# 1pathplanningzzj/pointnet_refine

Measured on AMD Instinct MI355X. Metric: lane segments/sec (fwd+bwd) at B=4096,N=1024; HBM GB/s vs roofline, higher is better.
Workload: dtype f32 (large GEMMs: 2xfp16-split MFMA, 3 products, fp32 accumulate); 1 GPU; LineRefineNet training step (fwd + deep-supervision L1 + bwd + Adam), B=4096/GPU, N=1024, M=32, C=4; global_batch=4096, points=1024, parallelism=dp1, decoder_chunk=4096

## Files before the change

include/pointnet_refine_hip.h:

```cpp
#ifndef POINTNET_REFINE_HIP_H
#define POINTNET_REFINE_HIP_H

#include <stddef.h>
#include <stdint.h>

#ifdef __cplusplus
extern "C" {
#endif

#define PRH_OK 0
#define PRH_ERR_ARG (-1)
#define PRH_ERR_WORKSPACE (-2)
#define PRH_ERR_HIP (-3)

#define PRH_MAX_LAYERS 8

typedef struct {
  const float* w;
  const float* b;
  const float* gamma;
  const float* beta;
  float* running_mean;
  float* running_var;
  int64_t* num_batches_tracked;
// ... 442 lines not shown
int prh_add_dropout_layernorm_forward(const float* x, const float* r, const float* gamma, const float* beta,
                                      long rows, int channels, float eps, float dropout_p, unsigned seed,
                                      float* y, float* mean, float* rstd, int device, void* stream);
size_t prh_add_dropout_layernorm_workspace_bytes(void);
int prh_add_dropout_layernorm_backward(const float* dy, const float* x, const float* r, const float* gamma,
                                       const float* mean, const float* rstd, long rows, int channels,
                                       float dropout_p, unsigned seed, float* dx, float* dr, float* dgamma,
                                       float* dbeta, void* workspace, size_t workspace_bytes, int device,
                                       void* stream);

size_t prh_l1_loss_workspace_bytes(void);
int prh_l1_loss(const float* pred, const float* target, int n_layers, long elems, double denom,
                int accumulate, float* loss, float* d_pred, float* geometry, double points,
                void* workspace, size_t workspace_bytes, int device, void* stream);

int prh_adam_step(float* param, const float* grad, float* exp_avg, float* exp_avg_sq, long n, float lr,
                  float beta1, float beta2, float eps, float weight_decay, int step, int device,
                  void* stream);

int prh_attn_backward_ex(const float* q, long ldq, const float* k, long ldk, const float* v, long ldv,
                         const float* o, long ldo, const float* lse, const float* dout, long lddo,
                         float* dq, long lddq, float* dk, long lddk, float* dv, long lddv, int B, int M,
                         int N, int H, float scale, float dropout_p, unsigned seed, float* kv_amax_part,
                         int device, void* stream);

int prh_set_gemm_mode(int mode);
int prh_get_gemm_mode(void);

int prh_set_dropout_seed_source(const unsigned* device_word);

int prh_test_gemm_nt(const float* a, const float* w, float* c, int m, int n, int k,
                     void* workspace, size_t workspace_bytes, int device, void* stream);
size_t prh_test_gemm_tn_workspace_bytes(int p, int mo, int ni);
size_t prh_test_gate_backward_workspace_bytes(int out_dim);
int prh_test_gate_backward(const float* ctx, int B, int N, int in_channel, int out_dim, const float* gate_w1,
                           const float* gate_b1, const float* gate_w2, const float* gate_b2, const float* z_fus,
                           const float* bn_scale, const float* bn_shift, float* d_fused, float* gate, int recompute,
                           float* ws_a, float* ws_b, void* workspace, size_t workspace_bytes, int device, void* stream);
int prh_test_gemm_tn(const float* a, const float* b, float* c, float* colsum, int p, int mo,
                     int ni, void* workspace, size_t workspace_bytes, int device, void* stream);
size_t prh_test_gemm_tn_side_workspace_bytes(int p, int mo, int ni);
int prh_test_gemm_tn_side(const float* a, const float* b, float* c, float* colsum, int p, int mo,
                          int ni, float* dy, long lddy, const float* z, long ldz, const float* ka,
                          const float* kb, const float* kc, long rows, int cols, int side,
                          float* amax_out, void* workspace, size_t workspace_bytes, int device,
                          void* stream);
int prh_test_gemm_tn_side_ex(const float* a, const float* b, float* c, float* colsum, int p, int mo,
                             int ni, const float* qa, const float* qb, float* dy, long lddy,
                             const float* z, long ldz, const float* ka, const float* kb,
                             const float* kc, long rows, int cols, int side, int period,
                             int* period_used, float* amax_out, void* workspace,
                             size_t workspace_bytes, int device, void* stream);

enum {
  PRH_REDUCE_SLABS = 0, PRH_REDUCE_BN_STAGE1 = 1, PRH_REDUCE_PARTIALS = 2, PRH_REDUCE_LN_PARAM_GRAD = 3,
  PRH_REDUCE_FINAL = 4, PRH_REDUCE_ACT_AMAX = 5
};
int prh_test_reduce_depth(int kind);
int prh_test_reduce_slabs(const float* slab, int s, int rows, int cols, float* out, long ldout,
                          const float* cslab, int ccols, float* cout, int device, void* stream);
int prh_test_reduce_bn_stage1(const float* ws_a, const float* ws_b, int r, long ld, int n,
                              int tile_rows, int p, int forward, double* out, int device,
                              void* stream);
int prh_test_reduce_partials(const float* ws_a, const float* ws_b, int r2, int n, float* out_a,
                             float* out_b, int device, void* stream);
int prh_test_reduce_ln_param_grad(const float* part_g, const float* part_b, int nb, float* dgamma,
// ... 25 lines not shown
```

pointnet_refine_amd/_lib.py:

```python
from __future__ import annotations

import ctypes as C
import os
import subprocess
import threading

_HERE = os.path.dirname(os.path.abspath(__file__))
_ROOT = os.path.dirname(_HERE)
LIB_PATH = os.environ.get("PRH_LIB_PATH") or os.path.join(_HERE, "libpointnet_refine_hip.so")
_CSRC = os.path.join(_HERE, "csrc")
_SOURCES = [os.path.join(_CSRC, "prh_lib.hip")] + (sorted(
    os.path.join(_CSRC, f) for f in os.listdir(_CSRC) if f.endswith((".hpp", ".h", ".hip")) and f != "prh_lib.hip")
    if os.path.isdir(_CSRC) else [])
_HEADER = os.path.join(_ROOT, "include", "pointnet_refine_hip.h")

PRH_MAX_LAYERS = 8


class BnLayer(C.Structure):
    _fields_ = [("w", C.c_void_p), ("b", C.c_void_p), ("gamma", C.c_void_p), ("beta", C.c_void_p),
                ("running_mean", C.c_void_p), ("running_var", C.c_void_p),
                ("num_batches_tracked", C.c_void_p), ("cin", C.c_int), ("cout", C.c_int)]


# ... 11 lines not shown
    _fields_ = [("conv", BnLayerGrad * 5), ("fusion", BnLayerGrad), ("d_gate_w1", C.c_void_p),
                ("d_gate_b1", C.c_void_p), ("d_gate_w2", C.c_void_p), ("d_gate_b2", C.c_void_p)]


class EncoderSaved(C.Structure):
    _fields_ = [("z_cat", C.c_void_p), ("z_fus", C.c_void_p), ("gate", C.c_void_p),
                ("bn_scale", C.c_void_p), ("bn_shift", C.c_void_p), ("bn_mean", C.c_void_p),
                ("bn_rstd", C.c_void_p), ("argmax", C.c_void_p), ("op_amax", C.c_void_p),
                ("gate_recompute", C.c_int)]


class EncoderSavedBf16(C.Structure):
    _fields_ = [("z_cat", C.c_void_p), ("z_fus", C.c_void_p), ("gate", C.c_void_p),
                ("bn_scale", C.c_void_p), ("bn_shift", C.c_void_p), ("bn_mean", C.c_void_p),
                ("bn_rstd", C.c_void_p), ("argmax", C.c_void_p)]


EXPORTS = [
    "prh_encoder_workspace_bytes", "prh_encoder_gate_recompute", "prh_encoder_forward", "prh_encoder_backward",
    "prh_encoder_bf16_workspace_bytes", "prh_encoder_forward_bf16", "prh_encoder_backward_bf16",
    "prh_linear_bf16_workspace_bytes", "prh_linear_forward_bf16", "prh_linear_backward_bf16",
    "prh_linear_forward_out16", "prh_linear_backward_dy16", "prh_attn_forward_kv16", "prh_attn_backward_kv16",
    "prh_encoder_fused_image_bytes", "prh_encoder_fused_prepare", "prh_encoder_fused_workspace_bytes",
    "prh_encoder_fused_forward",
    "prh_linear_forward_workspace_bytes", "prh_linear_forward", "prh_linear_forward_ex",
    "prh_linear_forward_full", "prh_linear_forward_amax", "prh_operand_absmax_workspace_bytes", "prh_operand_absmax",
    "prh_linear_uses_operand_maxima", "prh_linear_backward_full", "prh_linear_backward_amax", "prh_pos_hidden_forward",
    "prh_pos_hidden_forward_workspace_bytes", "prh_pos_hidden_forward_amax", "prh_pos_hidden_backward_workspace_bytes",
    "prh_pos_hidden_backward", "prh_linear_small_forward", "prh_linear_small_backward_workspace_bytes",
    "prh_linear_small_backward",
    "prh_linear_backward_workspace_bytes", "prh_linear_backward", "prh_linear_backward_ex",
    "prh_mlp_stack_workspace_bytes", "prh_mlp_stack_forward", "prh_mlp_stack_backward",
    "prh_test_gemm_nt", "prh_test_gemm_tn_workspace_bytes", "prh_test_gemm_tn",
    "prh_test_gate_backward_workspace_bytes", "prh_test_gate_backward",
    "prh_test_gemm_tn_side_workspace_bytes", "prh_test_gemm_tn_side", "prh_test_gemm_tn_side_ex", "prh_test_xcc_map",
    "prh_test_reduce_depth", "prh_test_reduce_slabs", "prh_test_reduce_bn_stage1", "prh_test_reduce_partials",
    "prh_test_reduce_ln_param_grad", "prh_test_reduce_pos_hidden_final", "prh_test_reduce_partial_rows_final",
    "prh_test_reduce_act_amax_workspace_bytes", "prh_test_reduce_act_amax",
    "prh_profile_enable", "prh_profile_count", "prh_profile_reset", "prh_profile_read",
    "prh_attn_forward", "prh_attn_backward", "prh_attn_backward_ex",
    "prh_context_workspace_bytes", "prh_context_build",
    "prh_context_ragged_workspace_bytes", "prh_context_ragged_count", "prh_context_ragged_select",
    "prh_line_metrics", "prh_shift_sweep_workspace_bytes", "prh_shift_sweep",
    "prh_shift_sweep_ragged_workspace_bytes", "prh_shift_sweep_ragged",
    "prh_drive_slice_workspace_bytes", "prh_drive_slice_count", "prh_drive_slice_write",
    "prh_drive_clip_workspace_bytes", "prh_drive_clip_count", "prh_drive_clip_write",
    "prh_drive_noise_workspace_bytes", "prh_drive_noise",
    "prh_match_clip_workspace_bytes", "prh_match_clip_count", "prh_match_clip_write",
    "prh_match_costs_workspace_bytes", "prh_match_costs", "prh_match_max_side", "prh_match_assign",
    "prh_bev_bounds_workspace_bytes", "prh_bev_bounds", "prh_bev_raster", "prh_bev_select_workspace_bytes",
    "prh_bev_select", "prh_bev_tone", "prh_bev_colorize", "prh_bev_crop", "prh_bev_tile", "prh_bev_draw_count",
    "prh_bev_draw_workspace_bytes", "prh_bev_draw",
    "prh_view_bounds_workspace_bytes", "prh_view_bounds", "prh_view_clear", "prh_view_max_views", "prh_view_splat",
    "prh_view_lines", "prh_view_resolve",
    "prh_fuse_max_points", "prh_fuse_tile", "prh_fuse_project_workspace_bytes", "prh_fuse_project",
    "prh_fuse_gather_workspace_bytes", "prh_fuse_gather",
    "prh_link_tile", "prh_link_pairs_per_block", "prh_link_pairs_workspace_bytes", "prh_link_pairs_count",
    "prh_link_pairs_write", "prh_link_stats",
    "prh_link_cum", "prh_link_edges_blocks", "prh_link_edges", "prh_link_edges_compact", "prh_link_label_round",
    "prh_link_tree_init", "prh_link_tree_level",
    "prh_support_max_cells", "prh_support_accumulate",
    "prh_ground_max_bins", "prh_ground_bin_workspace_bytes", "prh_ground_bin_count", "prh_ground_bin_write",
    "prh_ground_query",
    "prh_align_tile", "prh_align_max_shifts", "prh_align_select_workspace_bytes", "prh_align_select_count",
    "prh_align_select_write", "prh_align_score",
    "prh_align_max_poses", "prh_align_select_cells_workspace_bytes", "prh_align_select_cells_count",
# ... 298 lines not shown
    lib.prh_add_dropout_layernorm_backward.argtypes = [vp, vp, vp, vp, vp, vp, lg, i, f, C.c_uint, vp, vp, vp, vp,
                                                       vp, C.c_size_t, i, vp]
    lib.prh_l1_loss_workspace_bytes.restype = C.c_size_t
    lib.prh_l1_loss_workspace_bytes.argtypes = []
    lib.prh_l1_loss.restype = i
    lib.prh_l1_loss.argtypes = [vp, vp, i, lg, C.c_double, i, vp, vp, vp, C.c_double, vp, C.c_size_t, i, vp]
    lib.prh_adam_step.restype = i
    lib.prh_adam_step.argtypes = [vp, vp, vp, vp, lg, f, f, f, f, f, i, i, vp]
    lib.prh_cast_perm_bf16.restype = i
    lib.prh_cast_perm_bf16.argtypes = [vp, lg, vp, lg, i, vp]
    lib.prh_posmem_images.restype = i
    lib.prh_posmem_images.argtypes = [vp, lg, vp, vp, vp, vp, vp, lg, lg, vp, vp, i, vp]
    lib.prh_attn_fold_forward.restype = i
    lib.prh_attn_fold_forward.argtypes = [vp, lg, vp, vp, vp, lg, vp, lg, vp, vp, lg, i, i, i, i, C.c_float, i, vp]
    lib.prh_relu_mask_absmax.restype = i
    lib.prh_relu_mask_absmax.argtypes = [vp, vp, vp, lg, f, vp, vp, sz, i, vp]
    lib.prh_set_gemm_mode.restype = i
    lib.prh_set_gemm_mode.argtypes = [i]
    lib.prh_attn_backward_ex.restype = i
    lib.prh_attn_backward_ex.argtypes = [vp, lg, vp, lg, vp, lg, vp, lg, vp, vp, lg, vp, lg, vp, lg, vp, lg,
                                         i, i, i, i, f, f, C.c_uint, vp, i, vp]
    lib.prh_set_dropout_seed_source.restype = i
    lib.prh_set_dropout_seed_source.argtypes = [vp]
    lib.prh_get_gemm_mode.restype = i
    lib.prh_profile_enable.restype = i
    lib.prh_profile_enable.argtypes = [i]
    lib.prh_profile_count.restype = i
    lib.prh_profile_reset.restype = i
    lib.prh_profile_read.restype = i
    lib.prh_profile_read.argtypes = [i, C.c_char_p, i, C.POINTER(C.c_float), C.POINTER(C.c_double),
                                     C.POINTER(C.c_double)]
    lib.prh_test_gemm_nt.restype = i
    lib.prh_test_gemm_nt.argtypes = [vp, vp, vp, i, i, i, vp, sz, i, vp]
    lib.prh_test_gate_backward_workspace_bytes.restype = sz
    lib.prh_test_gate_backward_workspace_bytes.argtypes = [i]
    lib.prh_test_gate_backward.restype = i
    lib.prh_test_gate_backward.argtypes = [vp, i, i, i, i, vp, vp, vp, vp, vp, vp, vp, vp, vp, i, vp, vp, vp, sz, i, vp]
    lib.prh_test_gemm_tn_workspace_bytes.restype = sz
    lib.prh_test_gemm_tn_workspace_bytes.argtypes = [i, i, i]
    lib.prh_test_gemm_tn.restype = i
    lib.prh_test_gemm_tn.argtypes = [vp, vp, vp, vp, i, i, i, vp, sz, i, vp]
    lib.prh_test_gemm_tn_side_workspace_bytes.restype = sz
    lib.prh_test_gemm_tn_side_workspace_bytes.argtypes = [i, i, i]
    lib.prh_test_gemm_tn_side.restype = i
    lib.prh_test_gemm_tn_side.argtypes = [vp, vp, vp, vp, i, i, i, vp, lg, vp, lg, vp, vp, vp, lg, i, i, vp, vp, sz, i, vp]
    lib.prh_test_gemm_tn_side_ex.restype = i
    lib.prh_test_gemm_tn_side_ex.argtypes = [vp, vp, vp, vp, i, i, i, vp, vp, vp, lg, vp, lg, vp, vp, vp, lg, i, i, i,
                                             C.POINTER(i), vp, vp, sz, i, vp]
    lib.prh_test_xcc_map.restype = i
    lib.prh_test_xcc_map.argtypes = [i, i, vp, i, vp]
    if not hasattr(lib, "prh_test_reduce_depth"):
        return lib
    lib.prh_test_reduce_depth.restype = i
    lib.prh_test_reduce_depth.argtypes = [i]
    lib.prh_test_reduce_slabs.restype = i
    lib.prh_test_reduce_slabs.argtypes = [vp, i, i, i, vp, lg, vp, i, vp, i, vp]
    lib.prh_test_reduce_bn_stage1.restype = i
    lib.prh_test_reduce_bn_stage1.argtypes = [vp, vp, i, lg, i, i, i, i, vp, i, vp]
    lib.prh_test_reduce_partials.restype = i
    lib.prh_test_reduce_partials.argtypes = [vp, vp, i, i, vp, vp, i, vp]
    lib.prh_test_reduce_ln_param_grad.restype = i
    lib.prh_test_reduce_ln_param_grad.argtypes = [vp, vp, i, vp, vp, i, vp]
    lib.prh_test_reduce_pos_hidden_final.restype = i
    lib.prh_test_reduce_pos_hidden_final.argtypes = [vp, i, i, vp, vp, i, vp]
    lib.prh_test_reduce_partial_rows_final.restype = i
    lib.prh_test_reduce_partial_rows_final.argtypes = [vp, i, i, vp, i, vp, i, vp]
# ... 80 lines not shown
```

pointnet_refine_amd/csrc/prh_gemm_h2.hpp:

```cpp
#pragma once
#include "prh_gemm_s3.hpp"

namespace prh {

constexpr int H2_BK = 32;
constexpr int H2_PLANE = 256 * H2_BK * 2;
constexpr int H2_OPER = 2 * H2_PLANE;
constexpr int H2_STAGE = 2 * H2_OPER;
constexpr int H2_LDS = 2 * H2_STAGE;

__device__ __forceinline__ int h2_off(int row, int k) {
  return row * 64 + ((((k >> 3) ^ (-(row >> 2))) & 3) << 4) + ((k & 7) << 1);
}

inline size_t h2_weight_bytes(int N, int K) {
  return S3_WHDR + (size_t)((N + 255) / 256) * ((K + H2_BK - 1) / H2_BK) * H2_OPER;
}

__global__ __launch_bounds__(256) void prep_weights_h2_kernel(const float* __restrict__ W, int N,
                                                              int K, long ldw, char* __restrict__ out,
                                                              const float* __restrict__ amax) {
  const int KT = (K + H2_BK - 1) / H2_BK;
  const int NT_ = (N + 255) / 256;
  const long total = (long)NT_ * 256 * KT * 4;
// ... 292 lines not shown
      for (int r = 0; r < 4; ++r) acc[i][j][r] *= unscale;
  if constexpr (AMAX) {
    float wmax = 0.f;
    nt_epilogue_vec<EPI, 4, f32x4[8][4], false, true>(acc, p, m0 + wm, n0 + wn, tile_m * 2 + (wave >> 2), lane,
                                                       reinterpret_cast<float*>(smem) + wave * (32 * EPI_LDW), false, &wmax);
    __syncthreads();
    float* red = reinterpret_cast<float*>(smem);
    if (lane == 0) red[wave] = wmax;
    __syncthreads();
    if (tid == 0)
      p.ws_a[blockIdx.x] = fmaxf(fmaxf(fmaxf(red[0], red[1]), fmaxf(red[2], red[3])),
                                 fmaxf(fmaxf(red[4], red[5]), fmaxf(red[6], red[7])));
  } else if constexpr (EPI == EPI_GATE_BWD) {
    static_assert(8 * (32 + 16) * EPI_LDW * 4 <= H2_LDS, "gate-backward scratch must fit in the stage buffers");
    nt_epilogue_vec<EPI, 4>(acc, p, m0 + wm, n0 + wn, tile_m * 2 + (wave >> 2), lane,
                            reinterpret_cast<float*>(smem) + wave * (32 * EPI_LDW), false, nullptr,
                            reinterpret_cast<float*>(smem) + 8 * (32 * EPI_LDW) + wave * (16 * EPI_LDW));
  } else {
    nt_epilogue_vec<EPI, 4>(acc, p, m0 + wm, n0 + wn, tile_m * 2 + (wave >> 2), lane,
                            reinterpret_cast<float*>(smem) + wave * (32 * EPI_LDW));
  }
#ifdef PRH_STAMP
  PRH_TICK(2)
  asm volatile("s_waitcnt vmcnt(0)" ::: "memory");
  PRH_TICK(3)
  const int which = (p.K == 1024 && p.N == 1984) ? 0 : (p.K == 1984 && p.N == 1024) ? 1 : (p.K == 256 && p.N == 1536) ? 2 : (p.K == 512 && p.N == 1024) ? 3 : -1;
  if (g_prh_stamp != nullptr && which >= 0 && blockIdx.x == gridDim.x / 2 + 3 && lane == 0 && (wave & 3) == 0) {
    unsigned* o = g_prh_stamp + 64 + which * 16 + (wave >> 2) * 8;
#pragma unroll
    for (int i = 0; i < 4; ++i) o[i] = t_acc[i];
    o[4] = (unsigned)KT;
  }
#endif
}

typedef __fp16 fp16x4 __attribute__((__vector_size__(4 * sizeof(__fp16))));
constexpr int TR_ROW = 576;
constexpr int TR_PLANE = 16 * TR_ROW;
constexpr int TR_OPER = 2 * TR_PLANE;
constexpr int TR_STAGE = 2 * TR_OPER;
constexpr int TR_LDS = 2 * TR_STAGE;

__device__ __forceinline__ f16x8 tr_fragment(const char* plane, int col0, int lane) {
  const int g = lane >> 4, j = lane & 15;
  const char* a = plane + ((g >> 1) * 8 + (j >> 2)) * TR_ROW + (col0 + (g & 1) * 16 + 4 * (j & 3)) * 2;
  const fp16x4 lo = __builtin_amdgcn_ds_read_tr16_b64_v4f16(
      (__attribute__((address_space(3))) fp16x4*)(a));
  const fp16x4 hi = __builtin_amdgcn_ds_read_tr16_b64_v4f16(
      (__attribute__((address_space(3))) fp16x4*)(a + 4 * TR_ROW));
  struct Pair { fp16x4 a, b; } pr = {lo, hi};
  return __builtin_bit_cast(f16x8, pr);
}

constexpr int TR_PACE = 8;
constexpr int TR_PACE_SPINS = 256;
constexpr int TR_SIDE_MAX_COLS = 4096;
inline size_t tr_side_lds(int cols) { return (size_t)3 * ((cols + 255) / 256 * 256) * 4 + 64; }
typedef unsigned int u32x4 __attribute__((ext_vector_type(4)));

template <int PROB, bool SIDE = false, int Q = 1>
__global__ __launch_bounds__(512, 2) void gemm_tn_tr_kernel(const TNParams p) {
  static_assert(PROB == PRO_NONE || PROB == PRO_BNRELU, "prologue not supported");
  static_assert(Q == 1 || (SIDE && (Q == 2 || Q == 4)), "side period: 1, 2 or 4 k-tiles");
  extern __shared__ __attribute__((aligned(16))) char smem[];
  const int tid = threadIdx.x, lane = tid & 63, wave = tid >> 6;
  const int wm = (wave >> 2) * 128, wn = (wave & 3) * 64;
// ... 282 lines not shown
```

pointnet_refine_amd/csrc/prh_lib.hip:

```cpp
#include "../../include/pointnet_refine_hip.h"

#include <hip/hip_runtime.h>
#include <stdarg.h>
#include <stdio.h>
#include <string.h>

#include <mutex>
#include <vector>

#include <stdlib.h>

#include "prh_gemm.hpp"
#include "prh_attn.hpp"
#include "prh_attn16.hpp"
#include "prh_gemm_s3.hpp"
#include "prh_gemm_h2.hpp"
#include "prh_b16.hpp"
#include "prh_small.hpp"
#include "prh_attnfold.hpp"
#include "prh_fused.hpp"
#include "prh_context.hpp"
#include "prh_metrics.hpp"
#include "prh_drive.hpp"
#include "prh_match.hpp"
#include "prh_bev.hpp"
#include "prh_view.hpp"
#include "prh_fuse.hpp"
#include "prh_link.hpp"
#include "prh_link_sync.hpp"
#include "prh_support.hpp"
#include "prh_ground.hpp"
#include "prh_align.hpp"
#include "prh_trace.hpp"
#include "prh_pcd.hpp"
#include "prh_kernels.hpp"

using namespace prh;

namespace {
// ... 345 lines not shown
  const long tiles = (long)p.tiles_n * cdiv(p.M, TM * 32);
  char nm[64];
  snprintf(nm, sizeof(nm), "gemm_small<%d%d%d,%s,%d> K=%d N=%d", TM, TN, KS, NN ? "nn" : "nt", EPI, p.K, p.N);
  const double by = 4.0 * ((double)p.M * p.K + (double)p.M * p.N * ((p.flags & F_RESID) || EPI == EPI_DGRAD ? 2 : 1) + (double)p.N * p.K);
  ProfScope ps(nm, 2.0 * p.M * (double)p.N * p.K, by, st);
  hipLaunchKernelGGL((gemm_small_kernel<TM, TN, KS, NN, EPI>), dim3((unsigned)tiles), dim3(256), (small_lds<TM, TN, KS>()), st, p);
  LAUNCH_CHECK();
  return PRH_OK;
}
template <bool NN, int EPI = EPI_BIAS>
int launch_small(NTParams& p, hipStream_t st) {
  p.flags &= ~F_POOL;
  const bool n64 = !NN || (p.N & 63) == 0;
  if (n64 && (long)cdiv(p.M, 64) * cdiv(p.N, 64) >= 192) return launch_small_cfg<2, 2, 1, NN, EPI>(p, st);
  if (n64 && (long)cdiv(p.M, 32) * cdiv(p.N, 64) >= 192) return launch_small_cfg<1, 2, 2, NN, EPI>(p, st);
  return launch_small_cfg<1, 1, 4, NN, EPI>(p, st);
}
constexpr int TN_SMALL_MAX_P = 16384;
inline bool small_tn_dims_ok(int P, int Mo, int Ni) {
  return P >= 64 && P <= TN_SMALL_MAX_P && (P & 63) == 0 && (Mo & 63) == 0 && (Ni & 63) == 0;
}
inline void small_tn_plan(int P, int Mo, int Ni, int& splits, int& rps) {
  const int tiles = (Mo / 64) * (Ni / 64), chunks = P / 64;
  int s = cdiv(512, tiles);
  s = s > chunks ? chunks : (s < 1 ? 1 : s);
  rps = cdiv(chunks, s) * 64;
  splits = cdiv(P, rps);
}

inline size_t nt_amax_part_floats(int M, int N) {
  const size_t t = (size_t)cdiv(M < 1 ? 1 : M, S3_BM) * cdiv(N < 1 ? 1 : N, S3_BN);
  return (t > (size_t)ABSMAX_MAX_BLOCKS ? t : (size_t)ABSMAX_MAX_BLOCKS) + 64;
}
template <int PRO, int EPI>
int launch_nt_core(Cores c, NTParams& p, hipStream_t st, StatInfo* si, float* amax_part, long* amax_tiles) {
  if (p.M <= 0 || p.N <= 0) return PRH_OK;
  if ((p.K & 3) || (PRO != PRO_GATE1 && (p.lda & 3)) || (p.ldw & 3) ||
      (PRO == PRO_BNBWD && (p.lda2 & 3)))
    return fail(PRH_ERR_ARG, "gemm_nt: K/lda/ldw must be multiples of 4 (K=%d lda=%ld ldw=%ld)",
                p.K, p.lda, p.ldw);
  if constexpr (PRO == PRO_NONE && EPI == EPI_BIAS) {
    if (c.mode == 4 && c.core == 2 && nt_b16_generic_ok(p)) return launch_nt_b16<PRO_NONE, EPI_BIAS, false, false>(p, st, si);
  }
  const bool want_pool = (p.flags & F_POOL) != 0;
  p.flags &= ~F_POOL;
  char nm[64];
  const double by = 4.0 * ((double)p.M * p.K * (PRO == PRO_BNBWD ? 2 : (PRO == PRO_GATE1 ? 0 : 1)) +
                           (double)p.M * p.N * (EPI == EPI_GATE_BWD ? 4 : (EPI == EPI_GATE ? 3 : (EPI == EPI_DGRAD ? 2 : 1))) +
                           (double)p.N * p.K);
  {
    if (p.wprep != nullptr && nt_use_s3(c, p.M, p.N, p.K) && p.lda <= 65536 && p.lda2 <= 65536 &&
        !((EPI == EPI_GATE || EPI == EPI_GATE_BWD) && ((p.N | (int)p.ldc | (int)p.lde1 | (int)p.ldc2) & 3) != 0)) {
      const int KT = cdiv(p.K, S3_BK), NTl = cdiv(p.N, S3_BN);
      const long th = (long)NTl * 256 * KT * 2;
      float* hdr = reinterpret_cast<float*>(p.wprep);
      const char* img = p.wprep + S3_WHDR;
      if (c.core == 3) {
        if (p.amaxW == nullptr) {
          TRY_RC((measure_absmax<PRO_NONE>(p.W, p.ldw, nullptr, 0, nullptr, nullptr, nullptr, p.N, p.K, hdr, hdr + 64, st)));
          p.amaxW = hdr;
        }
        if (p.amaxA == nullptr) {
          TRY_RC((measure_absmax<PRO>(p.A, p.lda, p.A2, p.lda2, p.pa, p.pb, p.pc, p.M, p.K, hdr + 1, hdr + 64, st)));
          p.amaxA = hdr + 1;
        }
      }
      if constexpr (PRO == PRO_NONE || PRO == PRO_BNRELU || PRO == PRO_GATE1) {
        const bool vec_ok = ((p.N | (int)p.ldc) & 3) == 0 && (p.E1 == nullptr || ((int)p.lde1 & 3) == 0) &&
                            (p.flags & F_E1_ROWVEC) == 0 && (p.C2 == nullptr || ((int)p.ldc2 & 3) == 0);
        const int KT2 = cdiv(p.K, H2_BK);
        const size_t lds = (size_t)H2_LDS + (PRO == PRO_NONE ? 0 : 2 * (size_t)(KT2 + 2) * H2_BK * 4);
        if (c.core == 3 && vec_ok && lds <= 160 * 1024) {
          const long th2 = (long)NTl * 256 * KT2 * 4;
          hipLaunchKernelGGL(prep_weights_h2_kernel, dim3((unsigned)cdiv(th2, 256)), dim3(256), 0, st, p.W,
                             p.N, p.K, p.ldw, p.wprep + S3_WHDR, p.amaxW);
          LAUNCH_CHECK();
          p.tiles_n = NTl;
          if (want_pool) p.flags |= F_POOL;
          static const int attr_h2 = allow_big_lds(gemm_nt_h2_kernel<PRO, EPI>, gemm_nt_h2_kernel<PRO, EPI, true>);
          if (attr_h2 != PRH_OK) return attr_h2;
          snprintf(nm, sizeof(nm), "gemm_nt_h2<%d,%d> K=%d N=%d", PRO, EPI, p.K, p.N);
          ProfScope ps(nm, 2.0 * p.M * (double)p.N * p.K, by, st);
          if constexpr (PRO == PRO_NONE && EPI == EPI_BIAS) {
            if (amax_part != nullptr) {
              static const int attr_am = allow_big_lds(gemm_nt_h2_kernel<PRO, EPI, false, true>);
              if (attr_am != PRH_OK) return attr_am;
              const long wgs = (long)NTl * cdiv(p.M, 256);
              p.ws_a = amax_part;
              hipLaunchKernelGGL((gemm_nt_h2_kernel<PRO, EPI, false, true>), dim3((unsigned)wgs), dim3(512), lds, st, p, img);
              LAUNCH_CHECK();
              *amax_tiles = wgs;
              return PRH_OK;
            }
          }
          if (g_h2_pp)
            hipLaunchKernelGGL((gemm_nt_h2_kernel<PRO, EPI, true>), dim3((unsigned)(NTl * cdiv(p.M, 256))), dim3(512),
                               lds, st, p, img);
          else
            hipLaunchKernelGGL((gemm_nt_h2_kernel<PRO, EPI>), dim3((unsigned)(NTl * cdiv(p.M, 256))), dim3(512),
                               lds, st, p, img);
          LAUNCH_CHECK();
          if (si) { si->count = 2 * cdiv(p.M, S3_BM); si->rows = 128; }
          return PRH_OK;
        }
      }
      if constexpr (EPI != EPI_GATE_BWD) {
        hipLaunchKernelGGL(prep_weights_s3_kernel, dim3((unsigned)cdiv(th, 256)), dim3(256), 0, st,
                           p.W, p.N, p.K, p.ldw, 0, p.wprep + S3_WHDR, c.core == 3 ? p.amaxW : nullptr);
        LAUNCH_CHECK();
        p.tiles_n = NTl;
        const long tiles = (long)NTl * cdiv(p.M, S3_BM);
        static const int attr_rc = allow_big_lds(gemm_nt_s3_kernel<PRO, EPI, 3>, gemm_nt_s3_kernel<PRO, EPI, 1>,
                                                 gemm_nt_s3_kernel<PRO, EPI, 2>);
        if (attr_rc != PRH_OK) return attr_rc;
        snprintf(nm, sizeof(nm), "gemm_nt_%s<%d,%d> K=%d N=%d", c.core == 3 ? "h2g1" : c.tag(), PRO, EPI, p.K, p.N);
// ... 1 lines not shown
        switch (c.core) {
          case 2: launch_nt_s3<PRO, EPI, 1>(p, tiles, img, st); break;
          case 3: launch_nt_s3<PRO, EPI, 2>(p, tiles, img, st); break;
          default: launch_nt_s3<PRO, EPI, 3>(p, tiles, img, st);
        }
        LAUNCH_CHECK();
        if (si) { si->count = 2 * cdiv(p.M, S3_BM); si->rows = 128; }
        return PRH_OK;
      }
    }
  }
  if constexpr (EPI == EPI_GATE_BWD) {
    return fail(PRH_ERR_ARG, "gemm_nt: the gate-recompute backward needs the split-fp16 core (M=%d N=%d)", p.M, p.N);
  } else {
    if constexpr (PRO == PRO_NONE && EPI == EPI_BIAS) {
      if (small_nt_ok(p, false)) return launch_small<false>(p, st);
    }
    p.tiles_n = cdiv(p.N, BN);
    const long tiles = (long)p.tiles_n * cdiv(p.M, BM);
    snprintf(nm, sizeof(nm), "gemm_nt<%d,%d> K=%d N=%d", PRO, EPI, p.K, p.N);
    ProfScope ps(nm, 2.0 * p.M * (double)p.N * p.K, by, st);
    if (p.N <= 64)
      hipLaunchKernelGGL((gemm_nt_kernel<PRO, EPI, true>), dim3((unsigned)tiles), dim3(256), 0, st, p);
    else
      hipLaunchKernelGGL((gemm_nt_kernel<PRO, EPI>), dim3((unsigned)tiles), dim3(256), 0, st, p);
    LAUNCH_CHECK();
    if (si) { si->count = 2 * cdiv(p.M, BM); si->rows = 64; }
    return PRH_OK;
  }
}

template <int PRO, int EPI>
int launch_nt(Cores c, NTParams& p, hipStream_t st, StatInfo* si = nullptr, float* amax_out = nullptr,
              float* amax_part = nullptr) {
  long tiles = 0;
  TRY_RC((launch_nt_core<PRO, EPI>(c, p, st, si, amax_part, &tiles)));
  if (amax_out == nullptr) return PRH_OK;
  if (tiles > 0) {
    hipLaunchKernelGGL(absmax_final_kernel, dim3(1), dim3(256), 0, st, (const float*)amax_part, (int)tiles, amax_out);
    LAUNCH_CHECK();
    return PRH_OK;
  }
  return measure_absmax<PRO_NONE>(p.C, p.ldc, nullptr, 0, nullptr, nullptr, nullptr, p.M, p.N, amax_out, amax_part, st);
}

constexpr int TN_S3_MAX_LD = 4096;
struct TNPlan { int tiles_m, tiles_n, splits, rows_per_split; bool s3; };
inline TNPlan tn_plan(Cores c, int P, int Mo, int Ni, bool allow_s3, long maxld = TN_S3_MAX_LD) {
  TNPlan pl;
  pl.s3 = allow_s3 && tn_use_s3(c, P, Mo, Ni);
  const int tile = pl.s3 ? 256 : 128, bk = pl.s3 ? S3_BK : BK;
  pl.tiles_m = cdiv(Mo, tile);
  pl.tiles_n = cdiv(Ni, tile);
  const int tiles = pl.tiles_m * pl.tiles_n;
  int s = cdiv(pl.s3 ? (P >= 262144 ? 768 : 256) : 1024, tiles);
  if (pl.s3) {
    int best = s; double bw = 1e9;
    for (int c = (s > 3 ? s - 2 : 1); c <= s + 4; ++c) {
      const double blocks = (double)tiles * c, w = (double)cdiv((long)blocks, 256L) * 256.0 / blocks;
      if (w < bw - 1e-3) { bw = w; best = c; }
    }
    s = best;
  }
  const int minrows = pl.s3 ? 512 : 128;
  const int smax = cdiv(P, minrows) < 1 ? 1 : cdiv(P, minrows);
  if (s > smax) s = smax;
  if (s < 1) s = 1;
  int rps = cdiv(P, s);
  rps = cdiv(rps, bk) * bk;
// ... 3428 lines not shown
  }
  g_prof.on = true;
  return PRH_OK;
}
int prh_profile_count(void) {
  std::lock_guard<std::mutex> lk(g_prof.mu);
  return (int)g_prof.used;
}
int prh_profile_reset(void) {
  std::lock_guard<std::mutex> lk(g_prof.mu);
  g_prof.used = 0;
  return PRH_OK;
}
int prh_profile_read(int i, char* name, int name_len, float* ms, double* flops, double* bytes) {
  std::lock_guard<std::mutex> lk(g_prof.mu);
  if (i < 0 || (size_t)i >= g_prof.used) return fail(PRH_ERR_ARG, "profile_read: index %d out of range", i);
  ProfRec& r = g_prof.recs[(size_t)i];
  HIP_TRY(hipEventSynchronize(r.e1));
  HIP_TRY(hipEventElapsedTime(ms, r.e0, r.e1));
  snprintf(name, (size_t)name_len, "%s", r.name);
  *flops = r.flops; *bytes = r.bytes;
  return PRH_OK;
}

int prh_test_gemm_nt(const float* a, const float* w, float* c, int m, int n, int k, void* workspace,
                     size_t workspace_bytes, int device, void* stream) {
  HIP_TRY(hipSetDevice(device));
  NTParams p; memset(&p, 0, sizeof(p));
  p.A = a; p.lda = k; p.W = w; p.ldw = k; p.C = c; p.ldc = n; p.M = m; p.N = n; p.K = k;
  if (workspace != nullptr && workspace_bytes >= s3_weight_bytes(n, k) + 256)
    p.wprep = (char*)(((uintptr_t)workspace + 255) & ~(uintptr_t)255);
  return launch_nt<PRO_NONE, EPI_BIAS>(cores_of(gemm_mode()), p, (hipStream_t)stream);
}
size_t prh_test_gate_backward_workspace_bytes(int out_dim) { return s3_weight_bytes(out_dim, 64) + 512; }
int prh_test_gate_backward(const float* ctx, int B, int N, int in_channel, int out_dim, const float* gate_w1,
                           const float* gate_b1, const float* gate_w2, const float* gate_b2, const float* z_fus,
                           const float* bn_scale, const float* bn_shift, float* d_fused, float* gate, int recompute,
                           float* ws_a, float* ws_b, void* workspace, size_t workspace_bytes, int device, void* stream) {
  HIP_TRY(hipSetDevice(device));
  if (!ctx || !gate_w1 || !gate_b1 || !gate_w2 || !gate_b2 || !z_fus || !bn_scale || !bn_shift || !d_fused || !gate ||
      !ws_a || !ws_b || B <= 0 || N <= 0 || in_channel < 4 || out_dim <= 0 || (long)B * N > 2000000000L)
    return fail(PRH_ERR_ARG, "test_gate_backward: bad argument");
  const Cores c = cores_of(gemm_mode());
  if (recompute && !gate_on_h2(c, B * N, out_dim, in_channel))
    return fail(PRH_ERR_ARG, "test_gate_backward: recompute without prh_encoder_gate_recompute()");
  if (workspace == nullptr || workspace_bytes < prh_test_gate_backward_workspace_bytes(out_dim))
    return fail(PRH_ERR_WORKSPACE, "test_gate_backward: workspace too small");
  char* wprep = (char*)(((uintptr_t)workspace + 255) & ~(uintptr_t)255);
  return gate_combine_backward(c, ctx + 3, in_channel, B, N, out_dim, gate_w1, gate_b1, gate_w2, gate_b2, z_fus, bn_scale,
                               bn_shift, d_fused, nullptr, nullptr, gate, recompute, d_fused, ws_a, ws_b, wprep,
                               (hipStream_t)stream);
}
int prh_test_xcc_map(int blocks, int lds_bytes, int* out, int device, void* stream) {
  HIP_TRY(hipSetDevice(device));
  if (blocks <= 0 || lds_bytes < 0 || lds_bytes > 160 * 1024 || out == nullptr)
    return fail(PRH_ERR_ARG, "test_xcc_map: bad arguments");
  static const int attr_rc = allow_big_lds(xcc_probe_kernel);
  if (attr_rc != PRH_OK) return attr_rc;
  hipLaunchKernelGGL(xcc_probe_kernel, dim3((unsigned)blocks), dim3(512), (size_t)lds_bytes,
                     (hipStream_t)stream, out);
  LAUNCH_CHECK();
  return PRH_OK;
}
size_t prh_test_gemm_tn_workspace_bytes(int p, int mo, int ni) {
  const Cores c = cores_of(gemm_mode());
  Arena a;
// ... 137 lines not shown
```

Baseline: 10140 segments/s.

## Add persistent tile-walking h2 NT GEMM that prefetches next tile across epilogue

Adds a persistent variant of the fp16-split NT GEMM kernel for the bias epilogue with K up to 256. A grid sized to the CU count (rounded to a multiple of 8) walks over output tiles, and the loads of the next tile's first k-tiles are issued during the current tile's final iterations and epilogue. The aim is to hide the per-tile prologue and launch tail of short-K GEMMs. It is used automatically when tiles number at least twice the grid, and adds a test entry point. The cost is added complexity and shared-memory scratch reuse in the epilogue.

```diff
diff --git a/include/pointnet_refine_hip.h b/include/pointnet_refine_hip.h
--- a/include/pointnet_refine_hip.h
+++ b/include/pointnet_refine_hip.h
@@ -498,6 +498,11 @@
 int prh_test_gemm_nt(const float* a, const float* w, float* c, int m, int n, int k,
                      void* workspace, size_t workspace_bytes, int device, void* stream);
 size_t prh_test_gemm_tn_workspace_bytes(int p, int mo, int ni);
+size_t prh_test_gemm_nt_walk_workspace_bytes(int m, int n, int k);
+int prh_test_gemm_nt_walk(const float* a, const float* w, const float* bias, const float* e1, float* c, int m, int n,
+                          int k, int epilogue, int workgroups, const float* es, const float* et, float* stat_a,
+                          float* stat_b, float* amax_out, void* workspace, size_t workspace_bytes, int device,
+                          void* stream);
 size_t prh_test_gate_backward_workspace_bytes(int out_dim);
 int prh_test_gate_backward(const float* ctx, int B, int N, int in_channel, int out_dim, const float* gate_w1,
                            const float* gate_b1, const float* gate_w2, const float* gate_b2, const float* z_fus,
diff --git a/pointnet_refine_amd/_lib.py b/pointnet_refine_amd/_lib.py
--- a/pointnet_refine_amd/_lib.py
+++ b/pointnet_refine_amd/_lib.py
@@ -67,6 +67,7 @@
     "prh_linear_backward_workspace_bytes", "prh_linear_backward", "prh_linear_backward_ex",
     "prh_mlp_stack_workspace_bytes", "prh_mlp_stack_forward", "prh_mlp_stack_backward",
     "prh_test_gemm_nt", "prh_test_gemm_tn_workspace_bytes", "prh_test_gemm_tn",
+    "prh_test_gemm_nt_walk_workspace_bytes", "prh_test_gemm_nt_walk",
     "prh_test_gate_backward_workspace_bytes", "prh_test_gate_backward",
     "prh_test_gemm_tn_side_workspace_bytes", "prh_test_gemm_tn_side", "prh_test_gemm_tn_side_ex", "prh_test_xcc_map",
     "prh_test_reduce_depth", "prh_test_reduce_slabs", "prh_test_reduce_bn_stage1", "prh_test_reduce_partials",
@@ -431,6 +432,10 @@
                                      C.POINTER(C.c_double)]
     lib.prh_test_gemm_nt.restype = i
     lib.prh_test_gemm_nt.argtypes = [vp, vp, vp, i, i, i, vp, sz, i, vp]
+    lib.prh_test_gemm_nt_walk_workspace_bytes.restype = sz
+    lib.prh_test_gemm_nt_walk_workspace_bytes.argtypes = [i, i, i]
+    lib.prh_test_gemm_nt_walk.restype = i
+    lib.prh_test_gemm_nt_walk.argtypes = [vp, vp, vp, vp, vp, i, i, i, i, i, vp, vp, vp, vp, vp, vp, sz, i, vp]
     lib.prh_test_gate_backward_workspace_bytes.restype = sz
     lib.prh_test_gate_backward_workspace_bytes.argtypes = [i]
     lib.prh_test_gate_backward.restype = i
diff --git a/pointnet_refine_amd/csrc/prh_gemm_h2.hpp b/pointnet_refine_amd/csrc/prh_gemm_h2.hpp
--- a/pointnet_refine_amd/csrc/prh_gemm_h2.hpp
+++ b/pointnet_refine_amd/csrc/prh_gemm_h2.hpp
@@ -348,6 +348,166 @@
     o[4] = (unsigned)KT;
   }
 #endif
+}
+
+constexpr int H2W_SCR = 32 * EPI_LDW * 4;
+constexpr int H2W_LDS = H2_LDS + H2W_SCR;
+static_assert(7 * H2W_SCR <= H2_STAGE, "seven waves' epilogue scratch must fit in one stage");
+
+template <int EPI, bool AMAX = false>
+__global__ __launch_bounds__(512, 2) void gemm_nt_h2_walk_kernel(const NTParams p, const char* __restrict__ Wp,
+                                                                 const int tiles) {
+  static_assert(EPI == EPI_BIAS, "epilogue not supported");
+  extern __shared__ __attribute__((aligned(16))) char smem[];
+  const int KT = p.K / H2_BK;
+  const float sA = pow2_scale(load_amax(p.amaxA));
+  const float unscale = 1.f / (sA * pow2_scale(load_amax(p.amaxW)));
+  const unsigned lds0 = (unsigned)(unsigned long)((__attribute__((address_space(3))) char*)smem);
+
+  int par = 0;
+  f32x4 ra[2][4];
+  for (int v = blockIdx.x; v < tiles; v += gridDim.x) {
+    int tid = threadIdx.x;
+    asm volatile("" : "+v"(tid));
+    const int lane = tid & 63, wave = tid >> 6;
+    const int l15 = lane & 15, kc = lane >> 4;
+    const int wm = (wave >> 2) * 128, wn = (wave & 3) * 64;
+    const int sc = (tid & 7) * 4;
+    const int sr = tid >> 3;
+    const unsigned wdst = __builtin_amdgcn_readfirstlane(lds0 + H2_OPER + wave * 1024);
+    const int voA = (sr * (int)p.lda + sc) * 4;
+    const int rstep = 64 * (int)p.lda * 4;
+#ifdef PRH_STAMP
+    unsigned t_acc[4] = {0u, 0u, 0u, 0u};
+    unsigned long long t_prev = __builtin_amdgcn_s_memtime();
+#endif
+    const int vb = xcd_remap(v, tiles);
+    const int tile_n = vb % p.tiles_n, tile_m = vb / p.tiles_n;
+    const int m0 = tile_m * 256, n0 = tile_n * 256;
+    int arows = p.M - m0; arows = arows > 256 ? 256 : arows;
+    const int vn = v + (int)gridDim.x;
+    const bool more = vn < tiles;
+    const int vbn = xcd_remap(more ? vn : v, tiles);
+    const int mn = (vbn / p.tiles_n) * 256;
+    int arn = p.M - mn; arn = more ? (arn > 256 ? 256 : arn) : 0;
+    const size_t woff_own = (size_t)tile_n * KT * H2_OPER;
+    const size_t woff_next = more ? (size_t)(vbn % p.tiles_n) * KT * H2_OPER : woff_own + (size_t)(KT - 1) * H2_OPER;
+    f32x4 acc[8][4];
+    const char* wb = Wp + tid * 16;
+    auto dma_w = [&](int kt, int stage) {
+      const char* q = wb + (kt < KT ? woff_own + (size_t)kt * H2_OPER : woff_next);
+#pragma unroll
+      for (int pc = 0; pc < 4; ++pc) glds16(q + pc * 8192, wdst + stage * H2_STAGE + pc * 8192);
+    };
+    auto load_tile = [&](int kt, f32x4 (&r)[4]) {
+      const bool own = kt < KT;
+      const int nrows = own ? arows : arn;
+      const __amdgpu_buffer_rsrc_t rs = __builtin_amdgcn_make_buffer_rsrc(
+          (void*)(p.A + (size_t)(own ? m0 : mn) * p.lda), 0,
+          nrows > 0 ? (int)(((size_t)(nrows - 1) * p.lda + p.K) * 4) : 0, 0x00020000);
+      const int so = (own ? kt : kt - KT) * (H2_BK * 4);
+#pragma unroll
+      for (int j = 0; j < 4; ++j)
+        r[j] = __builtin_bit_cast(f32x4, __builtin_amdgcn_raw_buffer_load_b128(rs, voA, j * rstep + so, 0));
+    };
+    auto store_tile = [&](char* st, const f32x4 (&r_)[4]) {
+#pragma unroll
+      for (int j = 0; j < 4; ++j) {
+        const f32x4 x = r_[j] * sA;
+        uint2 h, l;
+        split2h(x[0], x[1], h.x, l.x);
+        split2h(x[2], x[3], h.y, l.y);
+        char* q = st + h2_off(sr + 64 * j, sc);
+        *reinterpret_cast<uint2*>(q) = h;
+        *reinterpret_cast<uint2*>(q + H2_PLANE) = l;
+      }
+    };
+    auto iter = [&](int kt, auto cs) {
+      constexpr int CS = decltype(cs)::value;
+      char* cur = smem + ((kt + par) & 1) * H2_STAGE;
+      char* nxt = smem + ((kt + 1 + par) & 1) * H2_STAGE;
+#pragma unroll
+      for (int j = 0; j < 4; ++j) asm volatile("" : "+v"(ra[CS][j]));
+      __builtin_amdgcn_sched_barrier(0);
+      dma_w(kt + 1, (kt + 1 + par) & 1);
+      __builtin_amdgcn_sched_barrier(0);
+      load_tile(kt + 2, ra[CS ^ 1]);
+      __builtin_amdgcn_sched_barrier(0);
+      h2_compute<0, 8>(acc, cur, wm, wn, l15, kc);
+      store_tile(nxt, ra[CS]);
+#pragma unroll
+      for (int g = 0; g < 48; ++g) {
+        __builtin_amdgcn_sched_group_barrier(0x008, 2, 0);
+        __builtin_amdgcn_sched_group_barrier(0x002, 3, 0);
+      }
+      asm volatile("s_waitcnt vmcnt(4)" ::: "memory");
+      __syncthreads();
+    };
+
+    if (v == (int)blockIdx.x) {
+      dma_w(0, 0);
+      __builtin_amdgcn_sched_barrier(0);
+      load_tile(0, ra[0]);
+      load_tile(1, ra[1]);
+      store_tile(smem, ra[0]);
+      asm volatile("s_waitcnt vmcnt(0)" ::: "memory");
+      __syncthreads();
+    }
+    PRH_TICK(0)
+#pragma unroll
+    for (int i = 0; i < 8; ++i)
+#pragma unroll
+      for (int j = 0; j < 4; ++j)
+#pragma unroll
+        for (int r = 0; r < 4; ++r) acc[i][j][r] = 0.f;
+    using I0 = std::integral_constant<int, 0>; using I1 = std::integral_constant<int, 1>;
+    int kt = 0;
+    for (; kt + 1 < KT; kt += 2) {
+      iter(kt, I1{});
+      iter(kt + 1, I0{});
+    }
+    if (kt < KT) iter(kt, I1{});
+    PRH_TICK(1)
+    const int sbase = ((KT - 1 + par) & 1) * H2_STAGE;
+    float* scr = reinterpret_cast<float*>(smem + (wave < 7 ? sbase + wave * H2W_SCR : H2_LDS));
+#pragma unroll
+    for (int i = 0; i < 8; ++i)
+#pragma unroll
+      for (int j = 0; j < 4; ++j)
+#pragma unroll
+        for (int r = 0; r < 4; ++r) acc[i][j][r] *= unscale;
+    if constexpr (AMAX) {
+      float wmax = 0.f;
+      nt_epilogue_vec<EPI, 4, f32x4[8][4], false, true>(acc, p, m0 + wm, n0 + wn, tile_m * 2 + (wave >> 2), lane, scr, false,
+                                                         &wmax);
+      __syncthreads();
+      float* red = reinterpret_cast<float*>(smem + sbase);
+      if (lane == 0) red[wave] = wmax;
+      __syncthreads();
+      if (tid == 0)
+        p.ws_a[v] = fmaxf(fmaxf(fmaxf(red[0], red[1]), fmaxf(red[2], red[3])),
+                          fmaxf(fmaxf(red[4], red[5]), fmaxf(red[6], red[7])));
+    } else {
+      nt_epilogue_vec<EPI, 4>(acc, p, m0 + wm, n0 + wn, tile_m * 2 + (wave >> 2), lane, scr);
+    }
+    PRH_TICK(2)
+    __syncthreads();
+    if (KT & 1) {
+#pragma unroll
+      for (int j = 0; j < 4; ++j) ra[1][j] = ra[0][j];
+    }
+    par = (KT + par) & 1;
+#ifdef PRH_STAMP
+    PRH_TICK(3)
+    if (g_prh_stamp != nullptr && p.K == 256 && p.N == 1536 && blockIdx.x == gridDim.x / 2 + 3 &&
+        v == (int)(blockIdx.x + 2 * gridDim.x) && lane == 0 && (wave & 3) == 0) {
+      unsigned* o = g_prh_stamp + 64 + 2 * 16 + (wave >> 2) * 8;
+#pragma unroll
+      for (int i = 0; i < 4; ++i) o[i] = t_acc[i];
+      o[4] = (unsigned)KT;
+    }
+#endif
+  }
 }
 
 typedef __fp16 fp16x4 __attribute__((__vector_size__(4 * sizeof(__fp16))));
diff --git a/pointnet_refine_amd/csrc/prh_lib.hip b/pointnet_refine_amd/csrc/prh_lib.hip
--- a/pointnet_refine_amd/csrc/prh_lib.hip
+++ b/pointnet_refine_amd/csrc/prh_lib.hip
@@ -5,6 +5,7 @@
 #include <stdio.h>
 #include <string.h>
 
+#include <atomic>
 #include <mutex>
 #include <vector>
 
@@ -416,8 +417,25 @@
   const size_t t = (size_t)cdiv(M < 1 ? 1 : M, S3_BM) * cdiv(N < 1 ? 1 : N, S3_BN);
   return (t > (size_t)ABSMAX_MAX_BLOCKS ? t : (size_t)ABSMAX_MAX_BLOCKS) + 64;
 }
+inline int device_cus() {
+  static std::atomic<int> cache[64];
+  int dev = 0;
+  if (hipGetDevice(&dev) != hipSuccess || dev < 0 || dev >= 64) return 0;
+  int cu = cache[dev].load(std::memory_order_relaxed);
+  if (cu == 0) {
+    if (hipDeviceGetAttribute(&cu, hipDeviceAttributeMultiprocessorCount, dev) != hipSuccess || cu <= 0) cu = -1;
+    cache[dev].store(cu, std::memory_order_relaxed);
+  }
+  return cu > 0 ? cu : 0;
+}
+constexpr int H2_WALK_MAX_K = 256;
+inline int nt_walk_grid(const NTParams& p, long tiles) {
+  if (g_h2_pp || p.K > H2_WALK_MAX_K || (p.K % H2_BK) != 0) return 0;
+  const int g = device_cus() & ~7;
+  return (g >= 8 && tiles >= 2L * g) ? g : 0;
+}
 template <int PRO, int EPI>
-int launch_nt_core(Cores c, NTParams& p, hipStream_t st, StatInfo* si, float* amax_part, long* amax_tiles) {
+int launch_nt_core(Cores c, NTParams& p, hipStream_t st, StatInfo* si, float* amax_part, long* amax_tiles, int walk = -1) {
   if (p.M <= 0 || p.N <= 0) return PRH_OK;
   if ((p.K & 3) || (PRO != PRO_GATE1 && (p.lda & 3)) || (p.ldw & 3) ||
       (PRO == PRO_BNBWD && (p.lda2 & 3)))
@@ -433,7 +451,7 @@
                            (double)p.M * p.N * (EPI == EPI_GATE_BWD ? 4 : (EPI == EPI_GATE ? 3 : (EPI == EPI_DGRAD ? 2 : 1))) +
                            (double)p.N * p.K);
   {
-    if (p.wprep != nullptr && nt_use_s3(c, p.M, p.N, p.K) && p.lda <= 65536 && p.lda2 <= 65536 &&
+    if (p.wprep != nullptr && (walk >= 0 || nt_use_s3(c, p.M, p.N, p.K)) && p.lda <= 65536 && p.lda2 <= 65536 &&
         !((EPI == EPI_GATE || EPI == EPI_GATE_BWD) && ((p.N | (int)p.ldc | (int)p.lde1 | (int)p.ldc2) & 3) != 0)) {
       const int KT = cdiv(p.K, S3_BK), NTl = cdiv(p.N, S3_BN);
       const long th = (long)NTl * 256 * KT * 2;
@@ -465,6 +483,25 @@
           if (attr_h2 != PRH_OK) return attr_h2;
           snprintf(nm, sizeof(nm), "gemm_nt_h2<%d,%d> K=%d N=%d", PRO, EPI, p.K, p.N);
           ProfScope ps(nm, 2.0 * p.M * (double)p.N * p.K, by, st);
+          if constexpr (PRO == PRO_NONE && EPI == EPI_BIAS) {
+            const long wtiles = (long)NTl * cdiv(p.M, 256);
+            const int wg = walk >= 0 ? walk : nt_walk_grid(p, wtiles);
+            if (wg > 0) {
+              static const int attr_wk = allow_big_lds(gemm_nt_h2_walk_kernel<EPI, false>, gemm_nt_h2_walk_kernel<EPI, true>);
+              if (attr_wk != PRH_OK) return attr_wk;
+              if (amax_part != nullptr) {
+                p.ws_a = amax_part;
+                hipLaunchKernelGGL((gemm_nt_h2_walk_kernel<EPI, true>), dim3((unsigned)wg), dim3(512), H2W_LDS, st, p, img, (int)wtiles);
+                LAUNCH_CHECK();
+                *amax_tiles = wtiles;
+                return PRH_OK;
+              }
+              hipLaunchKernelGGL((gemm_nt_h2_walk_kernel<EPI, false>), dim3((unsigned)wg), dim3(512), H2W_LDS, st, p, img, (int)wtiles);
+              LAUNCH_CHECK();
+              if (si) { si->count = 2 * cdiv(p.M, S3_BM); si->rows = 128; }
+              return PRH_OK;
+            }
+          }
           if constexpr (PRO == PRO_NONE && EPI == EPI_BIAS) {
             if (amax_part != nullptr) {
               static const int attr_am = allow_big_lds(gemm_nt_h2_kernel<PRO, EPI, false, true>);
@@ -532,9 +569,9 @@
 
 template <int PRO, int EPI>
 int launch_nt(Cores c, NTParams& p, hipStream_t st, StatInfo* si = nullptr, float* amax_out = nullptr,
-              float* amax_part = nullptr) {
+              float* amax_part = nullptr, int walk = -1) {
   long tiles = 0;
-  TRY_RC((launch_nt_core<PRO, EPI>(c, p, st, si, amax_part, &tiles)));
+  TRY_RC((launch_nt_core<PRO, EPI>(c, p, st, si, amax_part, &tiles, walk)));
   if (amax_out == nullptr) return PRH_OK;
   if (tiles > 0) {
     hipLaunchKernelGGL(absmax_final_kernel, dim3(1), dim3(256), 0, st, (const float*)amax_part, (int)tiles, amax_out);
@@ -4029,6 +4066,38 @@
     p.wprep = (char*)(((uintptr_t)workspace + 255) & ~(uintptr_t)255);
   return launch_nt<PRO_NONE, EPI_BIAS>(cores_of(gemm_mode()), p, (hipStream_t)stream);
 }
+size_t prh_test_gemm_nt_walk_workspace_bytes(int m, int n, int k) {
+  return align_up(s3_weight_bytes(n, k) + 512, 256) + nt_amax_part_floats(m, n) * sizeof(float) + 256;
+}
+int prh_test_gemm_nt_walk(const float* a, const float* w, const float* bias, const float* e1, float* c, int m, int n,
+                          int k, int epilogue, int workgroups, const float* es, const float* et, float* stat_a,
+                          float* stat_b, float* amax_out, void* workspace, size_t workspace_bytes, int device,
+                          void* stream) {
+  HIP_TRY(hipSetDevice(device));
+  if (!a || !w || !c || m <= 0 || n <= 0 || k < 2 * H2_BK || (k % H2_BK) != 0 || (n & 3) != 0 || epilogue < 0 ||
+      epilogue > 2 || workgroups < 0)
+    return fail(PRH_ERR_ARG, "test_gemm_nt_walk: bad argument (k in whole 32-deep k-tiles, n %% 4 == 0)");
+  if (epilogue == 2 && workgroups > 0)
+    return fail(PRH_ERR_ARG, "test_gemm_nt_walk: the walking form does not serve the dgrad epilogue");
+  if ((epilogue == 1 && !amax_out) || (epilogue == 2 && (!e1 || !es || !et || !stat_a || !stat_b)))
+    return fail(PRH_ERR_ARG, "test_gemm_nt_walk: the epilogue's operands are missing");
+  if (workspace == nullptr || workspace_bytes < prh_test_gemm_nt_walk_workspace_bytes(m, n, k))
+    return fail(PRH_ERR_WORKSPACE, "test_gemm_nt_walk: workspace too small (%zu bytes)", workspace_bytes);
+  const uintptr_t base = ((uintptr_t)workspace + 255) & ~(uintptr_t)255;
+  NTParams p; memset(&p, 0, sizeof(p));
+  p.A = a; p.lda = k; p.W = w; p.ldw = k; p.C = c; p.ldc = n; p.M = m; p.N = n; p.K = k; p.bias = bias;
+  p.wprep = (char*)base;
+  float* part = reinterpret_cast<float*>(base + align_up(s3_weight_bytes(n, k) + 512, 256));
+  const Cores cores{3, 3};
+  hipStream_t st = (hipStream_t)stream;
+  if (epilogue == 2) {
+    p.E1 = e1; p.lde1 = n; p.es = es; p.et = et; p.ws_a = stat_a; p.ws_b = stat_b; p.flags = F_MASK | F_STATS;
+    return launch_nt<PRO_NONE, EPI_DGRAD>(cores, p, st, nullptr, nullptr, nullptr, workgroups);
+  }
+  if (e1 != nullptr) { p.E1 = e1; p.lde1 = n; p.flags = F_RESID; }
+  return launch_nt<PRO_NONE, EPI_BIAS>(cores, p, st, nullptr, epilogue == 1 ? amax_out : nullptr,
+                                      epilogue == 1 ? part : nullptr, workgroups);
+}
 size_t prh_test_gate_backward_workspace_bytes(int out_dim) { return s3_weight_bytes(out_dim, 64) + 512; }
 int prh_test_gate_backward(const float* ctx, int B, int N, int in_channel, int out_dim, const float* gate_w1,
                            const float* gate_b1, const float* gate_w2, const float* gate_b2, const float* z_fus,
```

Result: no change. 10130 segments/s, median of 3 (-0.0%).
